# multi-template-matching/MultiTemplateMatching-Python

Measured on AMD Instinct MI355X. Metric: Mpixel-correlations/s, higher is better.
Workload: dtype u8

## Files before the change

include/mtm_hip.h:

```cpp
#ifndef MTM_HIP_H
#define MTM_HIP_H

#include <stddef.h>
#include <stdint.h>

#ifdef __cplusplus
extern "C" {
#endif

#define MTM_ABI_VERSION 9

#define MTM_U8  0
#define MTM_F32 1
#define MTM_U16 2

#define MTM_TM_SQDIFF        0
#define MTM_TM_SQDIFF_NORMED 1
#define MTM_TM_CCORR         2
#define MTM_TM_CCORR_NORMED  3
#define MTM_TM_CCOEFF        4
#define MTM_TM_CCOEFF_NORMED 5

#define MTM_PEAKS_LOCAL  0
#define MTM_PEAKS_GLOBAL 1
// ... 51 lines not shown
typedef struct mtm_point {
    int32_t templ_idx, x, y;
} mtm_point;

typedef struct mtm_timing {
    float total_ms;
    float score_ms;
    float peaks_ms;
    float ncc_kernel_ms;
    int32_t ncc_launches;
    int32_t kernel_used;
    int64_t n_hits;
    int32_t hits_only;
    float   sclk_mhz;
    float   ncc_sum_ms;
    int32_t f32_route;
    int32_t sq_launches;
    float   masked_stat_ms;
    int32_t f32_pieces;
} mtm_timing;

int         mtm_abi_version(void);
int         mtm_device_count(void);
const char* mtm_last_error(void);
int         mtm_ctx_create(mtm_ctx** out, int device_id);
void        mtm_ctx_destroy(mtm_ctx* ctx);
int         mtm_set_option(mtm_ctx* ctx, int option, int64_t value);
int         mtm_get_option(mtm_ctx* ctx, int option, int64_t* value);
#define MTM_POISON_SCRATCH 1
#define MTM_POISON_LDS     2
#define MTM_POISON_ARENAS  4
int         mtm_debug_poison(mtm_ctx* ctx, int pattern_byte, int what);
int         mtm_debug_quotient_check(mtm_ctx* ctx, uint64_t n_cases, uint64_t seed, uint64_t* out4);
int         mtm_debug_tail_split(int h, int w, double thr);
int         mtm_debug_templ_stats(const void* px, int rows, int cols, int chans, int dtype, int method, double* out7);
#define MTM_CLASS_TILING_FIELDS 13
int         mtm_debug_class_tilings(mtm_ctx* ctx, int32_t* out, int cap_classes);
int         mtm_debug_device_nms(mtm_ctx* ctx, const mtm_hit* hits, int64_t n, int rows, int cols, int max_side,
                                 double score_threshold, int ascending, double max_overlap, int64_t n_min, int64_t n_max,
                                 mtm_hit* out, int64_t capacity, int64_t* n_champions, int64_t* n_undecided);
#define MTM_PEAK_SCAN           0
#define MTM_PEAK_SCAN_BATCH     1
#define MTM_PEAK_SEGMENTS       2
#define MTM_PEAK_VERIFY_MAPS    3
#define MTM_PEAK_VERIFY_HASH    4
#define MTM_PEAK_EXTREMUM       5
#define MTM_PEAK_EXTREMUM_BATCH 6
typedef struct mtm_peak_pass {
    int32_t        n_maps, route, mode_min, border;
    float          thr, thr_q;
    int32_t        img_rows, holes, pattern_byte, reserved;
    int64_t        hit_cap;
    const int32_t* dims;
    const float*   maps;
    const uint8_t* flags;
    const mtm_hit* cands;
    int64_t        n_cands, cand_count, cand_cap;
    mtm_hit*       records;
    int64_t        capacity;
    uint64_t*      count;
    int32_t*       raw;
    int32_t*       trivial;
    int64_t        n_ints;
    uint64_t*      keys;
    mtm_hit*       ext_hits;
    uint64_t*      list_counts;
// ... 265 lines not shown
```

multitemplatematching-python_amd/MTM/_lib.py:

```python
import ctypes
import struct
import os
import threading
import weakref

import numpy as np

_HERE = os.path.dirname(os.path.abspath(__file__))
LIB_PATH = os.environ.get("MTM_LIB_PATH") or os.path.join(_HERE, "libmtm_hip.so")

MTM_U8, MTM_F32, MTM_U16 = 0, 1, 2
GROUP_EXCHANGE_HOST, GROUP_EXCHANGE_RCCL = 0, 1
PEAKS_LOCAL, PEAKS_GLOBAL = 0, 1
BORDER_CONSTANT, BORDER_NEAREST = 0, 1
KERNEL_AUTO, KERNEL_NAIVE, KERNEL_DOT4, KERNEL_MFMA = 0, 1, 2, 3
OPT_KERNEL, OPT_PEAK_BORDER, OPT_HIT_CAPACITY, OPT_DOT4_VARIANT, OPT_EXACT_DIV, OPT_HITS_ONLY, OPT_F32_MFMA = 1, 2, 3, 4, 5, 6, 7
OPT_BATCH_MAX_ROWS = 8
OPT_BOXES_MAX_FLOATS = 9
ALL_OPTIONS = (OPT_KERNEL, OPT_PEAK_BORDER, OPT_HIT_CAPACITY, OPT_DOT4_VARIANT, OPT_EXACT_DIV, OPT_HITS_ONLY, OPT_F32_MFMA,
               OPT_BATCH_MAX_ROWS, OPT_BOXES_MAX_FLOATS)
BATCH_MAX_ROWS = 65535
POISON_SCRATCH, POISON_LDS, POISON_ARENAS = 1, 2, 4
E_OVERFLOW = -5
E_HIP = -2
# ... 80 lines not shown
                ("want", ctypes.c_int32), ("sb0", ctypes.c_int32), ("sb1", ctypes.c_int32), ("lay_r0", ctypes.c_int32),
                ("lay_r1", ctypes.c_int32), ("pattern_byte", ctypes.c_int32),
                ("image", ctypes.c_void_p), ("t0", ctypes.c_void_p), ("t1", ctypes.c_void_p), ("t2", ctypes.c_void_p),
                ("t3", ctypes.c_void_p), ("sum2", ctypes.c_void_p), ("sq", ctypes.c_void_p), ("blk", ctypes.c_void_p),
                ("info", ctypes.c_void_p)]


MASKF32_SCREEN_INFO_FIELDS = ("n_templ", "h", "w", "oh", "ow", "nyb", "nseg", "mb", "cap_production", "cap", "count", "rescored")
MASKF32_CANARY = 8


class MtmMaskF32Screen(ctypes.Structure):
    _fields_ = [("pieces", ctypes.c_int32), ("mode", ctypes.c_int32), ("rescore", ctypes.c_int32), ("set_cap", ctypes.c_int32),
                ("thr", ctypes.c_float), ("reserved", ctypes.c_int32),
                ("list_cap", ctypes.c_int64),
                ("n_templ", ctypes.c_int64), ("oh", ctypes.c_int64), ("ow", ctypes.c_int64), ("tiles", ctypes.c_int64),
                ("c1", ctypes.c_void_p), ("c2", ctypes.c_void_p), ("lb", ctypes.c_void_p), ("ub", ctypes.c_void_p),
                ("map_listed", ctypes.c_void_p), ("map_rescored", ctypes.c_void_p), ("mu_i", ctypes.c_void_p),
                ("mu_j", ctypes.c_void_p), ("records", ctypes.c_void_p), ("capacity", ctypes.c_int64),
                ("best", ctypes.c_void_p), ("info", ctypes.c_void_p)]


_P = ctypes.POINTER
SYMBOLS = {
    "mtm_abi_version": (ctypes.c_int, []),
    "mtm_device_count": (ctypes.c_int, []),
    "mtm_last_error": (ctypes.c_char_p, []),
    "mtm_ctx_create": (ctypes.c_int, [_P(ctypes.c_void_p), ctypes.c_int]),
    "mtm_ctx_destroy": (None, [ctypes.c_void_p]),
    "mtm_set_option": (ctypes.c_int, [ctypes.c_void_p, ctypes.c_int, ctypes.c_int64]),
    "mtm_get_option": (ctypes.c_int, [ctypes.c_void_p, ctypes.c_int, _P(ctypes.c_int64)]),
    "mtm_debug_poison": (ctypes.c_int, [ctypes.c_void_p, ctypes.c_int, ctypes.c_int]),
    "mtm_debug_quotient_check": (ctypes.c_int, [ctypes.c_void_p, ctypes.c_uint64, ctypes.c_uint64, _P(ctypes.c_uint64)]),
    "mtm_debug_tail_split": (ctypes.c_int, [ctypes.c_int, ctypes.c_int, ctypes.c_double]),
    "mtm_debug_class_tilings": (ctypes.c_int, [ctypes.c_void_p, _P(ctypes.c_int32), ctypes.c_int]),
    "mtm_debug_templ_stats": (ctypes.c_int, [ctypes.c_void_p, ctypes.c_int, ctypes.c_int, ctypes.c_int, ctypes.c_int,
                                             ctypes.c_int, _P(ctypes.c_double)]),
    "mtm_debug_device_nms": (ctypes.c_int, [ctypes.c_void_p, ctypes.c_void_p, ctypes.c_int64, ctypes.c_int, ctypes.c_int,
                                            ctypes.c_int, ctypes.c_double, ctypes.c_int, ctypes.c_double, ctypes.c_int64,
                                            ctypes.c_int64, ctypes.c_void_p, ctypes.c_int64, _P(ctypes.c_int64),
                                            _P(ctypes.c_int64)]),
    "mtm_debug_peak_pass": (ctypes.c_int, [ctypes.c_void_p, ctypes.c_void_p]),
    "mtm_debug_window_stats": (ctypes.c_int, [ctypes.c_void_p, ctypes.c_void_p]),
    "mtm_debug_window_stats_route": (ctypes.c_int, [ctypes.c_void_p, ctypes.c_void_p]),
    "mtm_debug_maskf32_screen": (ctypes.c_int, [ctypes.c_void_p, ctypes.c_void_p]),
    "mtm_set_image": (ctypes.c_int, [ctypes.c_void_p, ctypes.c_void_p, ctypes.c_int, ctypes.c_int,
                                     ctypes.c_int, ctypes.c_int, ctypes.c_int64]),
    "mtm_set_image_downscaled": (ctypes.c_int, [ctypes.c_void_p, ctypes.c_void_p, ctypes.c_int, ctypes.c_int, ctypes.c_int,
                                                ctypes.c_int, ctypes.c_int64, ctypes.c_int]),
    "mtm_set_templates": (ctypes.c_int, [ctypes.c_void_p, ctypes.c_void_p, ctypes.c_int, ctypes.c_int]),
    "mtm_set_templates_augmented": (ctypes.c_int, [ctypes.c_void_p, ctypes.c_void_p, ctypes.c_int, ctypes.c_void_p, ctypes.c_int,
                                                   ctypes.c_int]),
    "mtm_score_map": (ctypes.c_int, [ctypes.c_void_p, ctypes.c_int, ctypes.c_void_p, ctypes.c_int64]),
    "mtm_find_matches": (ctypes.c_int, [ctypes.c_void_p, ctypes.c_int, ctypes.c_double, ctypes.c_void_p,
                                        ctypes.c_int64, _P(ctypes.c_int64)]),
    "mtm_find_matches_image": (ctypes.c_int, [ctypes.c_void_p, ctypes.c_void_p, ctypes.c_int, ctypes.c_int, ctypes.c_int,
                                              ctypes.c_int, ctypes.c_int64, ctypes.c_int, ctypes.c_double, ctypes.c_void_p,
                                              ctypes.c_int64, _P(ctypes.c_int64)]),
    "mtm_find_matches_image_nms": (ctypes.c_int, [ctypes.c_void_p, ctypes.c_void_p, ctypes.c_int, ctypes.c_int, ctypes.c_int,
                                                  ctypes.c_int, ctypes.c_int64, ctypes.c_double, ctypes.c_double, ctypes.c_int64,
                                                  ctypes.c_void_p, ctypes.c_int64, _P(ctypes.c_int64)]),
    "mtm_find_matches_image_sharded_nms": (ctypes.c_int, [ctypes.c_void_p, ctypes.c_void_p, ctypes.c_int, ctypes.c_int, ctypes.c_int,
                                                          ctypes.c_int, ctypes.c_int64, ctypes.c_double, ctypes.c_double,
                                                          ctypes.c_int64, ctypes.c_int, ctypes.c_void_p, ctypes.c_int,
                                                          ctypes.c_void_p, ctypes.c_int64, _P(ctypes.c_int64)]),
    "mtm_find_matches_batch": (ctypes.c_int, [ctypes.c_void_p, ctypes.c_void_p, ctypes.c_int, ctypes.c_int, ctypes.c_int,
# ... 482 lines not shown
    def __del__(self):
        try:
            self.close()
        except Exception:
            pass

    def set_option(self, opt, value):
        check(self._lib.mtm_set_option(self._h, int(opt), int(value)), "mtm_set_option")

    def get_option(self, opt):
        v = ctypes.c_int64(0)
        check(self._lib.mtm_get_option(self._h, int(opt), ctypes.byref(v)), "mtm_get_option")
        return int(v.value)

    def options(self):
        return {o: self.get_option(o) for o in ALL_OPTIONS}

    def debug_poison(self, pattern=0xFF, what=7):
        check(self._lib.mtm_debug_poison(self._h, int(pattern), int(what)), "mtm_debug_poison")

    def class_tilings(self):
        nf = len(CLASS_TILING_FIELDS)
        n = self._lib.mtm_debug_class_tilings(self._h, None, 0)
        check(min(n, 0), "mtm_debug_class_tilings")
        buf = (ctypes.c_int32 * (nf * max(n, 1)))()
        check(min(self._lib.mtm_debug_class_tilings(self._h, buf, n), 0), "mtm_debug_class_tilings")
        return [dict(zip(CLASS_TILING_FIELDS, buf[k * nf:(k + 1) * nf])) for k in range(n)]

    def debug_quotient_check(self, n_cases=1 << 28, seed=1):
        out = (ctypes.c_uint64 * 4)()
        check(self._lib.mtm_debug_quotient_check(self._h, int(n_cases), int(seed), out), "mtm_debug_quotient_check")
        return {"cases": int(out[0]), "mismatches": int(out[1]), "took_division": int(out[2]), "max_ulp_distance": int(out[3])}

    def debug_device_nms(self, hits, rows, cols, max_side, score_threshold, max_overlap, ascending=False, n_min=0,
                         n_max=1 << 18, out=None):
        hits = np.ascontiguousarray(hits, dtype=HIT_DTYPE)
        n = len(hits)
        if out is None:
            out = np.empty(max(n, 1), dtype=HIT_DTYPE)
        assert out.dtype == HIT_DTYPE and out.flags.c_contiguous
        nc, nu = ctypes.c_int64(0), ctypes.c_int64(0)
        check(self._lib.mtm_debug_device_nms(self._h, hits.ctypes.data, n, int(rows), int(cols), int(max_side),
                                             float(score_threshold), int(bool(ascending)), float(max_overlap), int(n_min),
                                             int(n_max), out.ctypes.data, len(out), ctypes.byref(nc), ctypes.byref(nu)),
              "mtm_debug_device_nms")
        return out[:nc.value], out[nc.value:nc.value + nu.value]

    def debug_peak_pass(self, maps, route, thr, mode_min=False, border=BORDER_NEAREST, hit_cap=4096, templ_hw=None, img_rows=0,
                        flags=None, holes=False, cands=None, cand_count=None, cand_cap=None, thr_q=None, pattern=0xFF,
                        records=None):
        maps = [np.ascontiguousarray(m, dtype=np.float32) for m in maps]
        n = len(maps)
        assert n >= 1 and all(m.ndim == 2 for m in maps)
        templ_hw = [(1, 1)] * n if templ_hw is None else list(templ_hw)
        dims = np.array([[m.shape[0], m.shape[1], hw[0], hw[1]] for m, hw in zip(maps, templ_hw)], dtype=np.int32)
        packed = np.concatenate([m.ravel() for m in maps])
        batch = route in (PEAK_SCAN_BATCH, PEAK_EXTREMUM_BATCH)
        n_img = (int(dims[0, 0]) + int(dims[0, 2]) - 1) // int(img_rows) if batch and img_rows > 0 else 1
        n_ints = n * max(n_img, 1)
        max_oh, max_ow = int(dims[:, 0].max()), int(dims[:, 1].max())
        n_sx = (max_ow + 255) // 256
        a = MtmPeakPass()
        a.n_maps, a.route, a.mode_min, a.border = n, int(route), int(bool(mode_min)), int(border)
        a.thr = float(thr)
        a.thr_q = float(thr_q) if thr_q is not None else float(np.float32(-np.float32(thr)) if mode_min else np.float32(thr))
        a.img_rows, a.holes, a.pattern_byte, a.hit_cap = int(img_rows), int(bool(holes)), int(pattern), int(hit_cap)
# ... 660 lines not shown
```

multitemplatematching-python_amd/csrc/mtm_k_stats.hip.h:

```cpp
#pragma once
#include <hip/hip_runtime.h>
#include <algorithm>
#include <cfloat>
#include <cstdint>

#include "mtm_kernels.h"
#include "../../include/mtm_hip.h"
#include "mtm_device_util.hip.h"

namespace mtm {

constexpr int kHsumSeg = 16;

template <typename AccT>
__global__ void hsum_kernel(const float* __restrict__ img, int pitch, long long plane, int rows,
                            int w, int ow, AccT* __restrict__ hs1, AccT* __restrict__ hs2,
                            int hs_pitch, long long hs_plane) {
    const int x0 = (blockIdx.x * blockDim.x + threadIdx.x) * kHsumSeg;
    const int y = blockIdx.y;
    const int c = blockIdx.z;
    if (x0 >= ow || y >= rows) return;
    const float* row = img + c * plane + (size_t)y * pitch;
    AccT s1 = 0, s2 = 0;
    for (int dx = 0; dx < w; ++dx) {
        const AccT v = (AccT)row[x0 + dx];
        s1 += v;
        s2 += v * v;
    }
    AccT* o1 = hs1 + c * hs_plane + (size_t)y * hs_pitch;
    AccT* o2 = hs2 + c * hs_plane + (size_t)y * hs_pitch;
    for (int k = 0; k < kHsumSeg; ++k) {
        const int x = x0 + k;
        if (x >= ow) break;
        o1[x] = s1;
        o2[x] = s2;
        const AccT vn = (AccT)row[x + w];
        const AccT vo = (AccT)row[x];
// ... 111 lines not shown

#ifndef MTM_STAT_BAND4
#define MTM_STAT_BAND4 8
#endif
constexpr int kStatBand4 = MTM_STAT_BAND4;
constexpr int kStatStrip = 1024;
#ifndef MTM_STAT_PRO_BATCH
#define MTM_STAT_PRO_BATCH 32
#endif
constexpr int kStatProBatch = MTM_STAT_PRO_BATCH;

inline int stats_u8_owg(int w) { return (kStatStrip + 1 - w) & ~15; }

struct StatLayout {
    uint8_t* u8 = nullptr;
    uint8_t* u8b = nullptr;
    int pitch = 0;
    int r0 = 0, r1 = 0;
    unsigned long long* zero16 = nullptr;
};

constexpr int kStatFormRows[] = {kStatBand4, 4};
constexpr int kStatFormCount = (int)(sizeof(kStatFormRows) / sizeof(kStatFormRows[0]));

inline int stats_u8_form(int strips, int units, int n_cus) {
    return (long long)strips * units <= 2ll * n_cus ? 2 : 1;
}

inline int stats_u8_grid_y(int sb0, int sb1, int oh, int rows_wg) {
    const int rows = std::min(sb1 * kStatBand4, oh) - sb0 * kStatBand4;
    return rows > 0 ? (rows + rows_wg - 1) / rows_wg : 0;
}

struct StatU8Args {
    const uint8_t* img = nullptr;
    int pitch = 0;
    int h = 0, w = 0, oh = 0, ow = 0;
    int num_type = 0, want_sq = 0, want_t = 0, want_sum2 = 0;
    double* t0 = nullptr;
    double* sum2 = nullptr;
    double* sq = nullptr;
    double* rsq = nullptr;
    int st_pitch = 0;
    double* blk = nullptr;
    double* blkq = nullptr;
    int blk_pitch = 0, tail_s = 0;
    int sb0 = 0, sb1 = 0;
    StatLayout lay;
    int owg = 0, rows_wg = kStatBand4;
    double inv_area = 0.0;
    double inv_nq[2] = {0.0, 0.0};
};

template <bool TAIL, bool RSQ>
__global__ __launch_bounds__(kStatStrip / 4) void stats_u8_kernel(const StatU8Args a) {
    constexpr int CPT = 4;
    constexpr int NT = kStatStrip / CPT;
    constexpr int NW = NT / 64;
    constexpr int BL = 16 / CPT;
    __shared__ __attribute__((aligned(16))) uint32_t E1[kStatStrip + 4], E2[kStatStrip + 4];
    constexpr int NS = TAIL ? 4 : 2;
    __shared__ __attribute__((aligned(16))) uint32_t wsum[NW][NS];
    __shared__ __attribute__((aligned(16))) uint32_t EQ1[TAIL ? kStatStrip + 4 : 4], EQ2[TAIL ? kStatStrip + 4 : 4];
    const uint8_t* __restrict__ img = a.img;
    const int pitch = a.pitch, h = a.h, w = a.w, ow = a.ow, owg = a.owg, st_pitch = a.st_pitch, tail_s = a.tail_s;
    const int x0 = blockIdx.x * owg, y0 = a.sb0 * kStatBand4 + (int)blockIdx.y * a.rows_wg;
    const int t = threadIdx.x, lane = t & 63, wave = __builtin_amdgcn_readfirstlane(t >> 6);
    const StatLayout& lay = a.lay;
    if (lay.zero16 != nullptr && blockIdx.x == 0 && blockIdx.y == 0 && t == 0) {
        lay.zero16[0] = 0ull;
        lay.zero16[1] = 0ull;
    }
    if (lay.u8b != nullptr) {
        const int nby = (int)gridDim.y, q = (lay.r1 - lay.r0 + nby - 1) / nby;
        const int ra = lay.r0 + (int)blockIdx.y * q, rb = min(lay.r1, ra + q);
        const int xe = blockIdx.x + 1 == gridDim.x ? pitch : min(pitch, x0 + owg);
        const int x = x0 + 4 * t;
        if (x < xe) {
            for (int r = ra; r < rb; r += 8) {
                uint32_t v[8];
#pragma unroll
                for (int i = 0; i < 8; ++i)
                    v[i] = r + i < rb ? *reinterpret_cast<const uint32_t*>(img + (size_t)(r + i) * pitch + x) : 0u;
#pragma unroll
                for (int i = 0; i < 8; ++i)
                    if (r + i < rb) {
                        const size_t o = (size_t)(r + i) * lay.pitch + x;
                        *reinterpret_cast<uint32_t*>(lay.u8 + o) = v[i];
                        *reinterpret_cast<uint32_t*>(lay.u8b + o) = v[i] ^ 0x80808080u;
                    }
            }
        }
    }
    const int y1 = min(min(a.sb1 * kStatBand4, a.oh), y0 + a.rows_wg);
    if (y0 >= y1) return;
    const int L = owg + w - 1;
    const int tc = CPT * t;
    const bool ld = (tc & ~3) < L && x0 + (tc | 3) < pitch;
    const uint8_t* base = img + (size_t)y0 * pitch + x0 + tc;
    auto load = [](const uint8_t* p) { return *reinterpret_cast<const uint32_t*>(p); };
    auto unpack = [](uint32_t v, uint32_t (&b)[CPT]) {
#pragma unroll
        for (int k = 0; k < CPT; ++k) b[k] = k == 3 ? v >> 24 : (v >> (8 * k)) & 255u;
    };
    uint32_t c1[CPT], c2[CPT];
    uint32_t q1[CPT], q2[CPT];
#pragma unroll
    for (int k = 0; k < CPT; ++k) c1[k] = c2[k] = q1[k] = q2[k] = 0u;
    for (int r0 = 0; r0 < h; r0 += kStatProBatch) {
        uint32_t v[kStatProBatch];
#pragma unroll
        for (int i = 0; i < kStatProBatch; ++i) v[i] = ld ? load(base + (size_t)min(r0 + i, h - 1) * pitch) : 0u;
#pragma unroll
        for (int i = 0; i < kStatProBatch; ++i)
            if (r0 + i < h) {
                uint32_t b[CPT];
                unpack(v[i], b);
#pragma unroll
                for (int k = 0; k < CPT; ++k) {
                    c1[k] += b[k];
                    c2[k] += b[k] * b[k];
                }
                if (TAIL && r0 + i >= tail_s) {
#pragma unroll
                    for (int k = 0; k < CPT; ++k) {
                        q1[k] += b[k];
                        q2[k] += b[k] * b[k];
                    }
                }
            }
    }
    const int xg = x0 + tc;
    const bool out_on = tc < owg && xg < st_pitch;
    const bool blk_on = (t & (BL - 1)) == 0 && tc < owg && (xg >> 4) < a.blk_pitch;
    for (int y = y0; y < y1; ++y) {
        uint32_t vn = 0, vo = 0, vq0 = 0, vq1 = 0;
        const bool odd = ((y - y0) & 1) != 0;
        if (y + 1 < y1 && ld) {
            vn = load(base + (size_t)(y - y0 + h) * pitch);
            vo = load(base + (size_t)(y - y0) * pitch);
            if (TAIL && odd) {
                vq0 = load(base + (size_t)(y - y0 + tail_s - 1) * pitch);
                vq1 = load(base + (size_t)(y - y0 + tail_s) * pitch);
            }
        }
        uint32_t s[NS], ws[NS];
        s[0] = s[1] = 0u;
#pragma unroll
        for (int k = 0; k < CPT; ++k) {
            s[0] += c1[k];
            s[1] += c2[k];
        }
        if constexpr (TAIL) {
            s[2] = s[3] = 0u;
#pragma unroll
            for (int k = 0; k < CPT; ++k) {
                s[2] += q1[k];
                s[3] += q2[k];
            }
        }
#pragma unroll
        for (int j = 0; j < NS; ++j) ws[j] = wave_inclusive_scan_u32(s[j]);
        if (lane == 63) {
#pragma unroll
            for (int j = 0; j < NS; ++j) wsum[wave][j] = ws[j];
        }
        __syncthreads();
        uint32_t off[NS];
#pragma unroll
        for (int j = 0; j < NS; ++j) off[j] = ws[j] - s[j];
#pragma unroll
        for (int k = 0; k < NW - 1; ++k)
            if (k < wave) {
#pragma unroll
                for (int j = 0; j < NS; ++j) off[j] += wsum[k][j];
            }
        uint32_t e1[CPT], e2[CPT], eq1[CPT], eq2[CPT];
        e1[0] = off[0];
        e2[0] = off[1];
#pragma unroll
        for (int k = 1; k < CPT; ++k) {
            e1[k] = e1[k - 1] + c1[k - 1];
            e2[k] = e2[k - 1] + c2[k - 1];
        }
#pragma unroll
        for (int k = 0; k < CPT; ++k) {
            E1[tc + k] = e1[k];
            E2[tc + k] = e2[k];
        }
        if (t == NT - 1) {
            E1[kStatStrip] = off[0] + s[0];
            E2[kStatStrip] = off[1] + s[1];
        }
        if constexpr (TAIL) {
            eq1[0] = off[2];
            eq2[0] = off[3];
#pragma unroll
            for (int k = 1; k < CPT; ++k) {
                eq1[k] = eq1[k - 1] + q1[k - 1];
                eq2[k] = eq2[k - 1] + q2[k - 1];
            }
#pragma unroll
            for (int k = 0; k < CPT; ++k) {
                EQ1[tc + k] = eq1[k];
                EQ2[tc + k] = eq2[k];
            }
            if (t == NT - 1) {
                EQ1[kStatStrip] = off[2] + s[2];
                EQ2[kStatStrip] = off[3] + s[3];
            }
        }
        __syncthreads();
        uint32_t lo = 0xffffffffu, hi = 0u;
        double sm = INFINITY;
        if (out_on) {
            double tt[CPT], ws2[CPT], sqv[CPT], rs[CPT];
#pragma unroll
            for (int k = 0; k < CPT; ++k) {
                const uint32_t s1 = E1[tc + k + w] - e1[k], s2 = E2[tc + k + w] - e2[k];
                tt[k] = (double)s1;
                ws2[k] = (double)s2;
                double wnd_mean2 = 0.0;
                if (a.num_type == 1) wnd_mean2 = (tt[k] * tt[k]) * a.inv_area;
                sqv[k] = window_norm(ws2[k], wnd_mean2);
                if constexpr (RSQ) rs[k] = sqv[k] > 0.0 ? 1.0 / sqv[k] : 0.0;
                if (xg + k < ow) {
                    lo = min(lo, s1);
                    hi = max(hi, s1);
                    sm = fmin(sm, sqv[k]);
                }
            }
            const size_t o = (size_t)y * st_pitch + xg;
            auto store = [&](double* plane, const double (&v)[CPT]) {
#pragma unroll
                for (int k = 0; k < CPT; k += 2) *reinterpret_cast<double2*>(plane + o + k) = make_double2(v[k], v[k + 1]);
            };
            if (a.want_t) store(a.t0, tt);
            if (a.want_sum2) store(a.sum2, ws2);
            if (a.want_sq) {
                store(a.sq, sqv);
                if constexpr (RSQ) store(a.rsq, rs);
            }
        }
        if (a.blk != nullptr) {
#pragma unroll
            for (int d = 1; d < BL; d <<= 1) {
                lo = min(lo, lane_group_xchg_u32(lo, d));
                hi = max(hi, lane_group_xchg_u32(hi, d));
                sm = fmin(sm, lane_group_xchg_f64(sm, d));
            }
            if (blk_on) {
                double* o = a.blk + ((size_t)y * a.blk_pitch + (xg >> 4)) * 4;
                *reinterpret_cast<double2*>(o) = make_double2(lo == 0xffffffffu ? 0.0 : (double)lo, (double)hi);
                *reinterpret_cast<double2*>(o + 2) = make_double2(sm, 0.0);
            }
        }
        if constexpr (TAIL) {
// ... 3 lines not shown
            if (out_on) {
#pragma unroll
                for (int k = 0; k < CPT; ++k)
                    if (xg + k < ow) {
                        const uint32_t s1q = EQ1[tc + k + w] - eq1[k], s2q = EQ2[tc + k + w] - eq2[k];
                        const double a1 = (double)s1q;
                        loq = min(loq, s1q);
                        hiq = max(hiq, s1q);
                        vm = fmax(vm, nq * (double)s2q - a1 * a1);
                    }
            }
#pragma unroll
            for (int d = 1; d < BL; d <<= 1) {
                loq = min(loq, lane_group_xchg_u32(loq, d));
                hiq = max(hiq, lane_group_xchg_u32(hiq, d));
                vm = fmax(vm, lane_group_xchg_f64(vm, d));
            }
            if (blk_on) {
                vm = sqrt(vm * a.inv_nq[odd ? 1 : 0]) * (1.0 + 0x1p-49);
                double* o = a.blkq + ((size_t)y * a.blk_pitch + (xg >> 4)) * 4;
                *reinterpret_cast<double2*>(o) = make_double2(loq == 0xffffffffu ? 0.0 : (double)loq, (double)hiq);
                *reinterpret_cast<double2*>(o + 2) = make_double2(vm, 0.0);
            }
        }
        uint32_t bn[CPT], bo[CPT];
        unpack(vn, bn);
        unpack(vo, bo);
#pragma unroll
        for (int k = 0; k < CPT; ++k) {
            c1[k] += bn[k] - bo[k];
            c2[k] += (uint32_t)__mul24((int)bn[k] - (int)bo[k], (int)(bn[k] + bo[k]));
        }
        if constexpr (TAIL) {
            uint32_t b0[CPT], b1[CPT];
            unpack(vq0, b0);
            unpack(vq1, b1);
#pragma unroll
            for (int k = 0; k < CPT; ++k) {
                q1[k] += bn[k] - b0[k] - b1[k];
                q2[k] += bn[k] * bn[k] - b0[k] * b0[k] - b1[k] * b1[k];
            }
        }
    }
}

__device__ __forceinline__ unsigned long long wave_inclusive_scan_u64(unsigned long long x, int lane) {
#pragma unroll
    for (int off = 1; off < 64; off <<= 1) {
        const unsigned long long y = __shfl_up(x, off);
        if (lane >= off) x += y;
    }
    return x;
}

__global__ __launch_bounds__(256) void stats_u16_kernel(const uint8_t* __restrict__ hib, const uint8_t* __restrict__ lob,
                                                        int pitch, int h, int w, int oh, int ow, int owg, double inv_area,
                                                        int num_type, int want_sq, int want_t, int want_sum2,
                                                        double* __restrict__ t0, double* __restrict__ sum2,
                                                        double* __restrict__ sq, int st_pitch,
                                                        double* __restrict__ blk = nullptr, int blk_pitch = 0, int yb_off = 0) {
    __shared__ __attribute__((aligned(16))) uint32_t E1[kStatStrip + 4];
    __shared__ __attribute__((aligned(16))) unsigned long long E2[kStatStrip + 4];
    __shared__ uint32_t wsum1[4];
    __shared__ unsigned long long wsum2[4];
    const int x0 = blockIdx.x * owg, y0 = ((int)blockIdx.y + yb_off) * kStatBand4;
    const int t = threadIdx.x, lane = t & 63, wave = t >> 6;
    const int L = owg + w - 1;
    const bool ld = 4 * t < L && x0 + 4 * t + 3 < pitch;
    const size_t base = (size_t)y0 * pitch + x0 + 4 * t;
    uint32_t c1[4] = {0, 0, 0, 0};
    unsigned long long c2[4] = {0, 0, 0, 0};
    auto px = [](uint32_t vh, uint32_t vl, uint32_t (&b)[4]) {
        vh ^= 0x80808080u;
// ... 386 lines not shown
```

multitemplatematching-python_amd/csrc/mtm_launch.hip:

```cpp
#include "mtm_ctx.h"

using namespace mtm;
using namespace mtmi;
#include "mtm_k_stats.hip.h"
#include "mtm_k_score.hip.h"
#include "mtm_refine.hip.h"
#include "mtm_maskf32.hip.h"

namespace {

struct DotVariant {
    int px, py, nt;
    bool wide;
    void (*fn)(DotParams, const TemplDev*, const int*, const uint8_t*, StatPlanes, float*);
};
#define DOTV(PX, PY, NT, W) {PX, PY, NT, W, ncc_dot4_kernel<PX, PY, NT, W>}
const DotVariant kDotVariants[] = {
    DOTV(4, 4, 4, false),
    DOTV(4, 4, 2, false),
    DOTV(8, 2, 4, false),
    DOTV(8, 4, 2, false),
    DOTV(4, 2, 4, false),
    DOTV(8, 2, 2, false),
    DOTV(4, 2, 8, false),
// ... 1541 lines not shown
    const int strips = (ow + stats_u8_owg(w) - 1) / stats_u8_owg(w);
    const int form = a->form ? a->form : stats_u8_form(strips, sb1 - sb0, n_cus);
    hipEvent_t ev[2] = {nullptr, nullptr};
    int rc = MTM_OK;
    float ms = 0.0f;
    hipError_t e = hipEventCreate(&ev[0]);
    if (e == hipSuccess) e = hipEventCreate(&ev[1]);
    if (e == hipSuccess) e = hipEventRecord(ev[0], c->stream);
    if (e == hipSuccess) rc = launch_stats_u8(c->stream, k, form, n_cus);
    if (e == hipSuccess && rc == MTM_OK) e = hipEventRecord(ev[1], c->stream);
    if (e == hipSuccess && rc == MTM_OK) e = hipStreamSynchronize(c->stream);
    if (e == hipSuccess && rc == MTM_OK) e = hipEventElapsedTime(&ms, ev[0], ev[1]);
    for (hipEvent_t v : ev)
        if (v) (void)hipEventDestroy(v);
    MTMC(rc);
    HIPC(e);
    const auto fetch = [&](void* to, size_t off, size_t bytes) -> int {
        if (to) HIPC(hipMemcpy(to, b + off, bytes, hipMemcpyDeviceToHost));
        return MTM_OK;
    };
    MTMC(fetch(a->t0, o_t0, st_bytes));
    MTMC(fetch(a->sum2, o_sum2, st_bytes));
    MTMC(fetch(a->sq, o_sq, st_bytes));
    MTMC(fetch(a->rsq, o_rsq, st_bytes));
    MTMC(fetch(a->blk, o_blk, rec_bytes));
    MTMC(fetch(a->blkq, o_blkq, rec_bytes));
    MTMC(fetch(a->u8, o_u8, (size_t)rows * pitch));
    MTMC(fetch(a->u8b, o_u8b, (size_t)rows * pitch));
    MTMC(fetch(a->header, o_hdr, 16));
    const int rows_wg = kStatFormRows[form - 1];
    const int64_t info[8] = {st_pitch, blk_pitch, pitch, form, strips, stats_u8_grid_y(sb0, sb1, oh, rows_wg), n_cus,
                             (int64_t)llround((double)ms * 1e6)};
    std::memcpy(a->info, info, sizeof(info));
    return MTM_OK;
}

int mtm_debug_window_stats_route(mtm_ctx* c, const mtm_window_stats_route* a) {
    if (!c || !a) {
        set_error("mtm_debug_window_stats_route: null context or arguments");
        return MTM_E_INVALID;
    }
    MTM_NOT_IN_FLIGHT(c, "mtm_debug_window_stats_route");
    const auto bad = [](const char* what) {
        set_error(std::string("mtm_debug_window_stats_route: ") + what);
        return MTM_E_INVALID;
    };
    const int rows = a->rows, cols = a->cols, chans = a->chans, h = a->h, w = a->w, dtype = a->dtype;
    if (!a->image || !a->info || rows < 1 || cols < 1 || rows > 16384 || cols > 16384 || h < 1 || w < 1 || h > rows || w > cols)
        return bad("an image of 1 .. 16384 rows and columns and a window inside it are needed");
    if (chans < 1 || chans > kMaxChans || (dtype != MTM_U8 && dtype != MTM_U16 && dtype != MTM_F32))
        return bad("1 .. 4 channels of uint8, uint16 or float32");
    if (a->num_type < 0 || a->num_type > 2 || a->pattern_byte < 0 || a->pattern_byte > 255 || a->route < 0 ||
        a->route >= kStatsRouteCount || (a->want & ~31) != 0)
        return bad("num_type 0 .. 2, a route, the planes wanted and a pattern byte");
    const int route = a->route ? a->route : (int)stats_route(dtype, chans, h, w, cols, true);
    if (route == kStatsRouteU8) return bad("the fused single-channel uint8 kernel is mtm_debug_window_stats's");
    if (const char* why = stats_route_refusal(route, dtype, chans, h, w, cols)) return bad(why);
    const StatGeom g = stat_geom(rows, cols, chans, h, w);
    const int oh = g.oh, ow = g.ow, nsb = (oh + kStatBand4 - 1) / kStatBand4;
    const int sb0 = a->sb0, sb1 = a->sb1 < 0 ? nsb : std::min(a->sb1, nsb);
    if (sb0 < 0 || sb0 >= sb1) return bad("an empty range of row units");
    const bool part = a->lay_r1 > a->lay_r0;
    const bool ranged = route == kStatsRouteU16 || (route == kStatsRouteF64Lds && part);
    if (part && route != kStatsRouteF64Lds) return bad("image rows lay_r0 .. lay_r1: the F64_LDS route only");
    if (!ranged && (sb0 != 0 || sb1 != nsb)) return bad("a range of row units: the U16 route or a partial F64_LDS launch only");
    const int o0 = sb0 * kStatBand4, o1 = std::min(oh, sb1 * kStatBand4);
// ... 220 lines not shown
```

Before: 410,700.

## Slim the u8 window-stats kernel with dot4 prologue, pointer walking and fast sqrt

The u8 window-statistics kernel now sums its prologue four rows at a time, transposing the bytes with perm and accumulating with udot4 instead of unpacking each byte. Row addresses are advanced by pointer increments rather than recomputed from indices. The tail-band accumulators are kept in negated form and updated with a pair-dot on odd rows. The library sqrt is replaced by an rsq-plus-Newton sqrt, with a new device check entry point that compares it bit for bit against sqrt. These changes aim to cut VALU and f64 instruction counts in the stats pass, at the cost of more intricate masking logic and reliance on the custom sqrt matching correctly rounded results.

```diff
diff --git a/include/mtm_hip.h b/include/mtm_hip.h
--- a/include/mtm_hip.h
+++ b/include/mtm_hip.h
@@ -107,6 +107,7 @@
 #define MTM_POISON_ARENAS  4
 int         mtm_debug_poison(mtm_ctx* ctx, int pattern_byte, int what);
 int         mtm_debug_quotient_check(mtm_ctx* ctx, uint64_t n_cases, uint64_t seed, uint64_t* out4);
+int         mtm_debug_sqrt_check(mtm_ctx* ctx, uint64_t n_triples, uint64_t seed, uint64_t n_integers, uint64_t* out4);
 int         mtm_debug_tail_split(int h, int w, double thr);
 int         mtm_debug_templ_stats(const void* px, int rows, int cols, int chans, int dtype, int method, double* out7);
 #define MTM_CLASS_TILING_FIELDS 13
diff --git a/multitemplatematching-python_amd/MTM/_lib.py b/multitemplatematching-python_amd/MTM/_lib.py
--- a/multitemplatematching-python_amd/MTM/_lib.py
+++ b/multitemplatematching-python_amd/MTM/_lib.py
@@ -136,6 +136,7 @@
     "mtm_get_option": (ctypes.c_int, [ctypes.c_void_p, ctypes.c_int, _P(ctypes.c_int64)]),
     "mtm_debug_poison": (ctypes.c_int, [ctypes.c_void_p, ctypes.c_int, ctypes.c_int]),
     "mtm_debug_quotient_check": (ctypes.c_int, [ctypes.c_void_p, ctypes.c_uint64, ctypes.c_uint64, _P(ctypes.c_uint64)]),
+    "mtm_debug_sqrt_check": (ctypes.c_int, [ctypes.c_void_p, ctypes.c_uint64, ctypes.c_uint64, ctypes.c_uint64, _P(ctypes.c_uint64)]),
     "mtm_debug_tail_split": (ctypes.c_int, [ctypes.c_int, ctypes.c_int, ctypes.c_double]),
     "mtm_debug_class_tilings": (ctypes.c_int, [ctypes.c_void_p, _P(ctypes.c_int32), ctypes.c_int]),
     "mtm_debug_templ_stats": (ctypes.c_int, [ctypes.c_void_p, ctypes.c_int, ctypes.c_int, ctypes.c_int, ctypes.c_int,
@@ -684,6 +685,11 @@
         check(self._lib.mtm_debug_quotient_check(self._h, int(n_cases), int(seed), out), "mtm_debug_quotient_check")
         return {"cases": int(out[0]), "mismatches": int(out[1]), "took_division": int(out[2]), "max_ulp_distance": int(out[3])}
 
+    def debug_sqrt_check(self, n_triples=1 << 28, seed=1, n_integers=1 << 24):
+        out = (ctypes.c_uint64 * 4)()
+        check(self._lib.mtm_debug_sqrt_check(self._h, int(n_triples), int(seed), int(n_integers), out), "mtm_debug_sqrt_check")
+        return {"compared": int(out[0]), "mismatches": int(out[1]), "guarded": int(out[2]), "worst_bits": int(out[3])}
+
     def debug_device_nms(self, hits, rows, cols, max_side, score_threshold, max_overlap, ascending=False, n_min=0,
                          n_max=1 << 18, out=None):
         hits = np.ascontiguousarray(hits, dtype=HIT_DTYPE)
diff --git a/multitemplatematching-python_amd/csrc/mtm_k_stats.hip.h b/multitemplatematching-python_amd/csrc/mtm_k_stats.hip.h
--- a/multitemplatematching-python_amd/csrc/mtm_k_stats.hip.h
+++ b/multitemplatematching-python_amd/csrc/mtm_k_stats.hip.h
@@ -3,6 +3,7 @@
 #include <algorithm>
 #include <cfloat>
 #include <cstdint>
+#include <type_traits>
 
 #include "mtm_kernels.h"
 #include "../../include/mtm_hip.h"
@@ -180,6 +181,40 @@
     return rows > 0 ? (rows + rows_wg - 1) / rows_wg : 0;
 }
 
+__device__ __forceinline__ void stat_transpose4(uint32_t r0, uint32_t r1, uint32_t r2, uint32_t r3, uint32_t (&col)[4]) {
+    const uint32_t a0 = __builtin_amdgcn_perm(r1, r0, 0x05010400u), a1 = __builtin_amdgcn_perm(r1, r0, 0x07030602u);
+    const uint32_t b0 = __builtin_amdgcn_perm(r3, r2, 0x05010400u), b1 = __builtin_amdgcn_perm(r3, r2, 0x07030602u);
+    col[0] = __builtin_amdgcn_perm(b0, a0, 0x05040100u);
+    col[1] = __builtin_amdgcn_perm(b0, a0, 0x07060302u);
+    col[2] = __builtin_amdgcn_perm(b1, a1, 0x05040100u);
+    col[3] = __builtin_amdgcn_perm(b1, a1, 0x07060302u);
+}
+__device__ __forceinline__ void stat_pair4(uint32_t r0, uint32_t r1, uint32_t (&pair)[4]) {
+    pair[0] = __builtin_amdgcn_perm(r1, r0, 0x0c0c0400u);
+    pair[1] = __builtin_amdgcn_perm(r1, r0, 0x0c0c0501u);
+    pair[2] = __builtin_amdgcn_perm(r1, r0, 0x0c0c0602u);
+    pair[3] = __builtin_amdgcn_perm(r1, r0, 0x0c0c0703u);
+}
+__device__ __forceinline__ uint32_t stat_rows_from(int n) {
+    return n <= 0 ? 0xffffffffu : n >= 4 ? 0u : 0xffffffffu << (8 * n);
+}
+__device__ __forceinline__ double stat_sqrt(double x) {
+    const double y = __builtin_amdgcn_rsq(x);
+    double g = x * y, hh = y * 0.5;
+    const double r = __builtin_fma(-hh, g, 0.5);
+    g = __builtin_fma(g, r, g);
+    hh = __builtin_fma(hh, r, hh);
+    const double d0 = __builtin_fma(-g, g, x);
+    g = __builtin_fma(d0, hh, g);
+    const double d1 = __builtin_fma(-g, g, x);
+    return __builtin_fma(d1, hh, g);
+}
+__device__ __forceinline__ double stat_window_norm(double sum2, double wnd_mean2) {
+    const double diff2 = fmax(sum2 - wnd_mean2, 0.0);
+    const bool small = diff2 <= fmin(0.5, (10.0 * (double)FLT_EPSILON) * sum2);
+    return small ? 0.0 : stat_sqrt(diff2);
+}
+
 struct StatU8Args {
     const uint8_t* img = nullptr;
     int pitch = 0;
@@ -245,39 +280,72 @@
     const int L = owg + w - 1;
     const int tc = CPT * t;
     const bool ld = (tc & ~3) < L && x0 + (tc | 3) < pitch;
-    const uint8_t* base = img + (size_t)y0 * pitch + x0 + tc;
-    auto load = [](const uint8_t* p) { return *reinterpret_cast<const uint32_t*>(p); };
+    const uint8_t* const row0 = img + (size_t)y0 * pitch + x0;
+    const size_t step = (size_t)pitch;
+    const uint32_t tcl = ld ? (uint32_t)tc : 0u;
+    auto load = [tcl](const uint8_t* row) { return *reinterpret_cast<const uint32_t*>(row + tcl); };
     auto unpack = [](uint32_t v, uint32_t (&b)[CPT]) {
 #pragma unroll
         for (int k = 0; k < CPT; ++k) b[k] = k == 3 ? v >> 24 : (v >> (8 * k)) & 255u;
     };
     uint32_t c1[CPT], c2[CPT];
-    uint32_t q1[CPT], q2[CPT];
-#pragma unroll
-    for (int k = 0; k < CPT; ++k) c1[k] = c2[k] = q1[k] = q2[k] = 0u;
-    for (int r0 = 0; r0 < h; r0 += kStatProBatch) {
+    uint32_t nq1[CPT], nq2[CPT];
+#pragma unroll
+    for (int k = 0; k < CPT; ++k) c1[k] = c2[k] = nq1[k] = nq2[k] = 0u;
+    static_assert(kStatProBatch % 4 == 0, "the prologue works on groups of four rows");
+    const uint8_t* pr = row0;
+    auto batch = [&](int r0, auto full) {
+        constexpr bool FULL = decltype(full)::value;
+        const int left = h - r0;
         uint32_t v[kStatProBatch];
 #pragma unroll
-        for (int i = 0; i < kStatProBatch; ++i) v[i] = ld ? load(base + (size_t)min(r0 + i, h - 1) * pitch) : 0u;
-#pragma unroll
-        for (int i = 0; i < kStatProBatch; ++i)
-            if (r0 + i < h) {
-                uint32_t b[CPT];
-                unpack(v[i], b);
+        for (int i = 0; i < kStatProBatch; ++i) {
+            v[i] = load(pr);
+            pr += FULL || i + 1 < left ? step : (size_t)0;
+        }
+#pragma unroll
+        for (int g = 0; g < kStatProBatch; g += 4)
+            if (FULL || g < left) {
+                uint32_t col[CPT];
+                stat_transpose4(v[g], v[g + 1], v[g + 2], v[g + 3], col);
+                if (!FULL && g + 4 > left) {
+                    const uint32_t keep = ~stat_rows_from(left - g);
+#pragma unroll
+                    for (int k = 0; k < CPT; ++k) col[k] &= keep;
+                }
 #pragma unroll
                 for (int k = 0; k < CPT; ++k) {
-                    c1[k] += b[k];
-                    c2[k] += b[k] * b[k];
-                }
-                if (TAIL && r0 + i >= tail_s) {
+                    c1[k] = __builtin_amdgcn_udot4(col[k], 0x01010101u, c1[k], false);
+                    c2[k] = __builtin_amdgcn_udot4(col[k], col[k], c2[k], false);
+                }
+                if (TAIL && (unsigned)(tail_s - r0 - g) < 4u) {
+                    const uint32_t keep = stat_rows_from(tail_s - r0 - g);
 #pragma unroll
                     for (int k = 0; k < CPT; ++k) {
-                        q1[k] += b[k];
-                        q2[k] += b[k] * b[k];
+                        const uint32_t cq = col[k] & keep;
+                        nq1[k] = c1[k] - __builtin_amdgcn_udot4(cq, 0x01010101u, 0u, false);
+                        nq2[k] = c2[k] - __builtin_amdgcn_udot4(cq, cq, 0u, false);
                     }
                 }
             }
-    }
+    };
+    int r0 = 0;
+    for (; r0 + kStatProBatch <= h; r0 += kStatProBatch) batch(r0, std::true_type{});
+    if (r0 < h) batch(r0, std::false_type{});
+    if (TAIL && (unsigned)tail_s < (unsigned)h) {
+#pragma unroll
+        for (int k = 0; k < CPT; ++k) {
+            nq1[k] -= c1[k];
+            nq2[k] -= c2[k];
+        }
+    }
+    if (!ld) {
+#pragma unroll
+        for (int k = 0; k < CPT; ++k) c1[k] = c2[k] = nq1[k] = nq2[k] = 0u;
+    }
+    const uint8_t* pn = row0 + (size_t)h * step;
+    const uint8_t* po = row0;
+    const uint8_t* pq = row0 + (size_t)(TAIL ? tail_s - 1 : 0) * step;
     const int xg = x0 + tc;
     const bool out_on = tc < owg && xg < st_pitch;
     const bool blk_on = (t & (BL - 1)) == 0 && tc < owg && (xg >> 4) < a.blk_pitch;
@@ -285,13 +353,16 @@
         uint32_t vn = 0, vo = 0, vq0 = 0, vq1 = 0;
         const bool odd = ((y - y0) & 1) != 0;
         if (y + 1 < y1 && ld) {
-            vn = load(base + (size_t)(y - y0 + h) * pitch);
-            vo = load(base + (size_t)(y - y0) * pitch);
+            vn = load(pn);
+            vo = load(po);
             if (TAIL && odd) {
-                vq0 = load(base + (size_t)(y - y0 + tail_s - 1) * pitch);
-                vq1 = load(base + (size_t)(y - y0 + tail_s) * pitch);
-            }
-        }
+                vq0 = load(pq);
+                vq1 = load(pq + step);
+            }
+        }
+        pn += step;
+        po += step;
+        pq += step;
         uint32_t s[NS], ws[NS];
         s[0] = s[1] = 0u;
 #pragma unroll
@@ -303,8 +374,8 @@
             s[2] = s[3] = 0u;
 #pragma unroll
             for (int k = 0; k < CPT; ++k) {
-                s[2] += q1[k];
-                s[3] += q2[k];
+                s[2] -= nq1[k];
+                s[3] -= nq2[k];
             }
         }
 #pragma unroll
@@ -345,8 +416,8 @@
             eq2[0] = off[3];
 #pragma unroll
             for (int k = 1; k < CPT; ++k) {
-                eq1[k] = eq1[k - 1] + q1[k - 1];
-                eq2[k] = eq2[k - 1] + q2[k - 1];
+                eq1[k] = eq1[k - 1] - nq1[k - 1];
+                eq2[k] = eq2[k - 1] - nq2[k - 1];
             }
 #pragma unroll
             for (int k = 0; k < CPT; ++k) {
@@ -370,7 +441,7 @@
                 ws2[k] = (double)s2;
                 double wnd_mean2 = 0.0;
                 if (a.num_type == 1) wnd_mean2 = (tt[k] * tt[k]) * a.inv_area;
-                sqv[k] = window_norm(ws2[k], wnd_mean2);
+                sqv[k] = stat_window_norm(ws2[k], wnd_mean2);
                 if constexpr (RSQ) rs[k] = sqv[k] > 0.0 ? 1.0 / sqv[k] : 0.0;
                 if (xg + k < ow) {
                     lo = min(lo, s1);
@@ -440,13 +511,19 @@
             c2[k] += (uint32_t)__mul24((int)bn[k] - (int)bo[k], (int)(bn[k] + bo[k]));
         }
         if constexpr (TAIL) {
-            uint32_t b0[CPT], b1[CPT];
-            unpack(vq0, b0);
-            unpack(vq1, b1);
 #pragma unroll
             for (int k = 0; k < CPT; ++k) {
-                q1[k] += bn[k] - b0[k] - b1[k];
-                q2[k] += bn[k] * bn[k] - b0[k] * b0[k] - b1[k] * b1[k];
+                nq1[k] -= bn[k];
+                nq2[k] -= bn[k] * bn[k];
+            }
+            if (odd) {
+                uint32_t pair[CPT];
+                stat_pair4(vq0, vq1, pair);
+#pragma unroll
+                for (int k = 0; k < CPT; ++k) {
+                    nq1[k] = __builtin_amdgcn_udot4(pair[k], 0x01010101u, nq1[k], false);
+                    nq2[k] = __builtin_amdgcn_udot4(pair[k], pair[k], nq2[k], false);
+                }
             }
         }
     }
diff --git a/multitemplatematching-python_amd/csrc/mtm_launch.hip b/multitemplatematching-python_amd/csrc/mtm_launch.hip
--- a/multitemplatematching-python_amd/csrc/mtm_launch.hip
+++ b/multitemplatematching-python_amd/csrc/mtm_launch.hip
@@ -1597,6 +1597,92 @@
     const int64_t info[8] = {st_pitch, blk_pitch, pitch, form, strips, stats_u8_grid_y(sb0, sb1, oh, rows_wg), n_cus,
                              (int64_t)llround((double)ms * 1e6)};
     std::memcpy(a->info, info, sizeof(info));
+    return MTM_OK;
+}
+
+}
+
+namespace mtmi {
+
+__device__ __forceinline__ uint64_t sc_mix(uint64_t z) {
+    z += 0x9E3779B97F4A7C15ull;
+    z = (z ^ (z >> 30)) * 0xBF58476D1CE4E5B9ull;
+    z = (z ^ (z >> 27)) * 0x94D049BB133111EBull;
+    return z ^ (z >> 31);
+}
+__global__ __launch_bounds__(256) void sqrt_check_kernel(uint64_t n_per_thread, uint64_t seed, uint64_t n_int, unsigned long long* out) {
+    const uint64_t gid = (uint64_t)blockIdx.x * blockDim.x + threadIdx.x, nthreads = (uint64_t)gridDim.x * blockDim.x;
+    unsigned long long n = 0, bad = 0, guarded = 0, worst = 0;
+    const auto compare = [&](double x) {
+        const unsigned long long a = (unsigned long long)__double_as_longlong(stat_sqrt(x));
+        const unsigned long long b = (unsigned long long)__double_as_longlong(sqrt(x));
+        ++n;
+        if (a != b) {
+            ++bad;
+            const unsigned long long xb = (unsigned long long)__double_as_longlong(x);
+            worst = xb > worst ? xb : worst;
+        }
+    };
+    const auto guarded_compare = [&](double sum2, double mean2) {
+        const double diff2 = fmax(sum2 - mean2, 0.0);
+        if (diff2 <= fmin(0.5, (10.0 * (double)FLT_EPSILON) * sum2)) ++guarded;
+        else compare(diff2);
+    };
+    for (uint64_t k = 0; k < n_per_thread; ++k) {
+        const uint64_t idx = gid * n_per_thread + k;
+        const uint64_t r0 = sc_mix(seed ^ (idx * 4u)), r1 = sc_mix(seed ^ (idx * 4u + 1u)), r2 = sc_mix(seed ^ (idx * 4u + 2u));
+        uint64_t area = 1u + r0 % 66051u;
+        if (r0 & (1ull << 40)) area = 1u + area % (1u << (1u + (unsigned)((r0 >> 41) % 16u)));
+        const uint64_t s1 = r1 % (255u * area + 1u);
+        uint64_t s2;
+        if ((idx & 1u) == 0u) {
+            s2 = r2 % (65025u * area + 1u);
+        } else {
+            const uint64_t lo = (s1 * s1 + area - 1u) / area, hi = 255u * s1;
+            s2 = lo + r2 % (hi - lo + 1u);
+        }
+        const double t = (double)s1, inv_area = 1.0 / (double)area;
+        guarded_compare((double)s2, (t * t) * inv_area);
+        guarded_compare((double)s2, 0.0);
+    }
+    for (uint64_t k = 1u + gid; k <= n_int; k += nthreads) {
+        const double x = (double)k;
+        compare(x);
+        compare(__longlong_as_double(__double_as_longlong(x) - 1));
+        compare(__longlong_as_double(__double_as_longlong(x) + 1));
+    }
+    atomicAdd(&out[0], n);
+    atomicAdd(&out[1], bad);
+    atomicAdd(&out[2], guarded);
+    atomicMax(&out[3], worst);
+}
+
+}
+
+extern "C" {
+
+int mtm_debug_sqrt_check(mtm_ctx* c, uint64_t n_triples, uint64_t seed, uint64_t n_integers, uint64_t* out4) {
+    if (!c || !out4) {
+        set_error("mtm_debug_sqrt_check: null context or output");
+        return MTM_E_INVALID;
+    }
+    MTM_NOT_IN_FLIGHT(c, "mtm_debug_sqrt_check");
+    if (n_triples > (1ull << 36) || n_integers > (1ull << 32)) {
+        set_error("mtm_debug_sqrt_check: at most 2^36 triples and 2^32 integers");
+        return MTM_E_INVALID;
+    }
+    HIPC(hipSetDevice(c->device));
+    const int blocks = 2048, threads = 256;
+    const uint64_t per = (n_triples + (uint64_t)blocks * threads - 1) / ((uint64_t)blocks * threads);
+    MTMC(c->stats_dbg.ensure(256));
+    unsigned long long* acc = c->stats_dbg.as<unsigned long long>();
+    HIPC(hipMemsetAsync(acc, 0, 4 * sizeof(unsigned long long), c->stream));
+    hipLaunchKernelGGL(mtmi::sqrt_check_kernel, dim3(blocks), dim3(threads), 0, c->stream, per, seed, n_integers, acc);
+    HIPC(hipGetLastError());
+    unsigned long long h[4] = {0, 0, 0, 0};
+    HIPC(hipMemcpyAsync(h, acc, sizeof(h), hipMemcpyDeviceToHost, c->stream));
+    HIPC(hipStreamSynchronize(c->stream));
+    for (int i = 0; i < 4; ++i) out4[i] = h[i];
     return MTM_OK;
 }
 
diff --git a/profiles/stats_kernel_diet/count_loop.py b/profiles/stats_kernel_diet/count_loop.py
--- /dev/null
+++ b/profiles/stats_kernel_diet/count_loop.py
@@ -0,0 +1,52 @@
+#!/usr/bin/env python3
+import re
+import sys
+
+
+def cls(op):
+    if "_dpp" in op:
+        return "dpp"
+    if op.startswith("ds_"):
+        return "lds"
+    if op.startswith(("global_", "flat_", "buffer_", "scratch_")):
+        return "vmem"
+    if op.startswith("v_"):
+        return "f64" if "f64" in op else "valu"
+    return "salu"
+
+
+def main(path, prefix):
+    lines = open(path).read().split("\n")
+    start = next(i for i, l in enumerate(lines) if l.startswith(prefix) and ":" in l)
+    end = next(i for i in range(start, len(lines)) if lines[i].startswith(".Lfunc_end"))
+    body = lines[start:end]
+    bars = [i for i, l in enumerate(body) if l.strip().startswith("s_barrier")]
+    assert len(bars) == 2, bars
+    head = max(i for i in range(bars[0]) if "Loop Header" in body[i])
+    label = body[head].split(":")[0].lstrip(".L")
+    counts = {"row loop": {}, "outside the row loop": {}}
+    where = "outside the row loop"
+    for i, l in enumerate(body):
+        if re.match(r"^\.LBB\d+_\d+:", l) or re.match(r"^; %bb\.", l):
+            text = l + " " + (body[i + 1] if i + 1 < len(body) and body[i + 1].lstrip().startswith(";") else "")
+            inside = i == head or re.search(r"Header=" + label + r"\b", text) is not None
+            where = "row loop" if inside else "outside the row loop"
+            continue
+        if re.match(r"^\s+[a-z]+_[a-z0-9_]+", l) is None:
+            continue
+        op = l.split()[0]
+        n = counts[where]
+        if op == "s_nop":
+            n["nops"] = n.get("nops", 0) + int(l.split()[1]) + 1
+            continue
+        if op == "s_waitcnt":
+            continue
+        n[cls(op)] = n.get(cls(op), 0) + 1
+    print(lines[start].split(":")[0])
+    for name, n in counts.items():
+        total = sum(v for k, v in n.items() if k != "nops")
+        print("  %-22s total %4d  %s" % (name, total, "  ".join("%s %d" % kv for kv in sorted(n.items()))))
+
+
+if __name__ == "__main__":
+    main(sys.argv[1], sys.argv[2])
diff --git a/profiles/stats_kernel_diet/trace_summary.py b/profiles/stats_kernel_diet/trace_summary.py
--- /dev/null
+++ b/profiles/stats_kernel_diet/trace_summary.py
@@ -0,0 +1,13 @@
+#!/usr/bin/env python3
+import sqlite3
+import sys
+
+con = sqlite3.connect(sys.argv[1])
+cols = [d[0] for d in con.execute("select * from kernels limit 0").description]
+gy = "grid_y" if "grid_y" in cols else "0"
+like = "%" + (sys.argv[2] if len(sys.argv) > 2 else "") + "%"
+rows = con.execute("select name, grid_x, %s, workgroup_x, count(*), avg(duration)/1e3, min(duration)/1e3, max(duration)/1e3 "
+                   "from kernels where name like ? group by name, grid_x, %s order by sum(duration) desc" % (gy, gy), (like,)).fetchall()
+print("kernel,grid_x,grid_y,workgroup_x,calls,avg_us,min_us,max_us")
+for r in rows:
+    print("%s,%d,%d,%d,%d,%.2f,%.2f,%.2f" % ((r[0].replace(",", ";"),) + tuple(r[1:])))
```

Result: no change. 415,600, median of 4 (+1.2%).
